# bluecube/minipath

Measured on AMD Instinct MI355X. Metric: Mrays/s, higher is better.
Workload: dtype f32; 1 GPU; atrium stand-in for the absent data/Sponza (reference .gitmodules:1-3: un-fetched submodule), 258432 triangles, generator seed 1; 1920x1080 256spp tile64 seed0x5eed depth1 (reference semantics: primary ray + |d.n|, worker.rs:51-66); parallelism=tiles round-robin over 1 rank(s)

## Files before the change

minipath_amd/csrc/family_launch.h:

```cpp
#pragma once

#include <hip/hip_runtime.h>

#include <string>
#include <type_traits>

#include "launch_plan.h"
#include "mp_internal.h"

namespace mp {

#pragma GCC visibility push(hidden)
int check(hipError_t e, const char* what, std::string& err);
void note_launch(KernelId id);
int launched(KernelId id, std::string& err);
int launch_tiles(const RenderLaunch& L, const LaunchPlan& plan, hipStream_t st, std::string& err);
int launch_paths(const RenderLaunch& L, const LaunchPlan& plan, hipStream_t st, std::string& err);
int launch_aov(const RenderLaunch& L, const mp_aov_planes_ex& planes, const LaunchPlan& plan, hipStream_t st, std::string& err);
int launch_staged(const RenderLaunch& L, const WavefrontPlan& plan, hipStream_t st, std::string& err);
int launch_rays(QueryKind kind, const DevScene& sc, const float* ox, const float* oy, const float* oz, const float* dx, const float* dy,
                const float* dz, const float* tmax, uint64_t n, const mp_hits_soa* hits, uint8_t* occluded, int cu_count, void* stream,
                std::string& err);
#ifdef MP_PROF_MISSES
constexpr int kProfSlots = 10;
int prof_add_tiles(unsigned long long* sum, int reset);
int prof_add_aov(unsigned long long* sum, int reset);
int prof_add_paths(unsigned long long* sum, int reset);
#endif
#pragma GCC visibility pop

#define MP_LAUNCH(id, kernel, grid, block, lds, stream, ...)               \
    do {                                                                   \
        note_launch(id);                                                   \
        hipLaunchKernelGGL(kernel, grid, block, lds, stream, __VA_ARGS__); \
    } while (0)

#define MP_LAUNCH_ROW(row, ...)                                                          \
    case row:                                                                            \
        if constexpr (std::is_invocable_v<decltype(&__VA_ARGS__), Args...>) {            \
            MP_LAUNCH(row, (__VA_ARGS__), dim3(grid), dim3(block), lds, st, args...);    \
            return launched(row, err);                                                   \
        }                                                                                \
        break;
#define MP_FAMILY_LAUNCHER(SUBTABLE)                                                                                              \
    template <class... Args>                                                                                                      \
    int launch(KernelId id, uint32_t grid, uint32_t block, uint32_t lds, hipStream_t st, std::string& err, const Args&... args) { \
        switch (id) {                                                                                                             \
            SUBTABLE(MP_LAUNCH_ROW)                                                                                               \
            default: break;                                                                                                       \
        }                                                                                                                         \
        err = "kernel table: no such kernel for these arguments";                                                                 \
        return MP_ERR_INVALID;                                                                                                    \
    }

namespace {

template <class Plan>
int refused(const Plan& plan, std::string& err) {
    err = plan.error;
    return plan.rc;
}

}
}
```

minipath_amd/csrc/mask_cache.h:

```cpp
#pragma once

#include <hip/hip_runtime.h>

#include <cfloat>
#include <cmath>
#include <cstdint>

#include "camera_rays.h"

#ifndef MP_PROF_COUNT
#define MP_PROF_COUNT(i) do { } while (0)
#endif

namespace mp {
namespace mc {
__device__ __forceinline__ float as_f(uint32_t u) { return __uint_as_float(u); }
__device__ __forceinline__ uint32_t as_u(float f) { return __float_as_uint(f); }

__device__ __forceinline__ void wave_lds_sync() {
    __builtin_amdgcn_fence(__ATOMIC_RELEASE, "wavefront");
    __builtin_amdgcn_wave_barrier();
    __builtin_amdgcn_fence(__ATOMIC_ACQUIRE, "wavefront");
}

struct Ray {
    float ox, oy, oz, dx, dy, dz, ix, iy, iz;
};

__device__ __forceinline__ float fma_dot(float ax, float ay, float az, float bx, float by, float bz) {
    return __builtin_fmaf(az, bz, __builtin_fmaf(ay, by, ax * bx));
}
__device__ __forceinline__ float fms(float a, float b, float c) { return __builtin_fmaf(a, b, -c); }

template <bool PATCH_NAN, int OCT>
__device__ __forceinline__ void slab(float bnx, float bny, float bnz, float bxx, float bxy, float bxz, const Ray& r,
                                     float limit, float& t1, float& t2) {
    float ax = (bnx - r.ox) * r.ix, ay = (bny - r.oy) * r.iy, az = (bnz - r.oz) * r.iz;
    float cx = (bxx - r.ox) * r.ix, cy = (bxy - r.oy) * r.iy, cz = (bxz - r.oz) * r.iz;
    if (PATCH_NAN) {
        ax = fmaxf(ax, -INFINITY); ay = fmaxf(ay, -INFINITY); az = fmaxf(az, -INFINITY);
        cx = fminf(cx, INFINITY); cy = fminf(cy, INFINITY); cz = fminf(cz, INFINITY);
    }
    float lox, loy, loz, hix, hiy, hiz;
    if (OCT >= 0) {
        lox = (OCT & 1) ? cx : ax; hix = (OCT & 1) ? ax : cx;
        loy = (OCT & 2) ? cy : ay; hiy = (OCT & 2) ? ay : cy;
        loz = (OCT & 4) ? cz : az; hiz = (OCT & 4) ? az : cz;
    } else {
        lox = fminf(ax, cx); loy = fminf(ay, cy); loz = fminf(az, cz);
        hix = fmaxf(ax, cx); hiy = fmaxf(ay, cy); hiz = fmaxf(az, cz);
    }
    t1 = fmaxf(fmaxf(lox, 0.0f), fmaxf(loy, loz));
    t2 = fminf(fminf(hix, limit), fminf(hiy, hiz));
}

#ifndef MP_MCACHE_PAD
#define MP_MCACHE_PAD 0.25f
#endif
#ifndef MP_NODE_ENTRIES
#define MP_NODE_ENTRIES 64
#endif
#ifndef MP_LEAF_ENTRIES
#define MP_LEAF_ENTRIES 128
#endif
#ifndef MP_ARENA_ENTRIES
#define MP_ARENA_ENTRIES 384
#endif
#ifndef MP_ARENA_ROOM
#define MP_ARENA_ROOM 384
#endif
#ifndef MP_NODE_SLOT_MASK
#define MP_NODE_SLOT_MASK 0xFFFFFFFFu
#endif
constexpr int kMaskCacheEntries = MP_NODE_ENTRIES;
constexpr int kMaskCacheHeader = 32;
constexpr int kLeafCacheEntries = MP_LEAF_ENTRIES;
constexpr int kLeafTagBase = kMaskCacheHeader + kMaskCacheEntries;
constexpr int kLeafMaskBase = kLeafTagBase + kLeafCacheEntries;
constexpr int kNodeListBase = kLeafMaskBase + 2 * kLeafCacheEntries;
constexpr int kArenaBase = kNodeListBase + kMaskCacheEntries;
constexpr int kArenaRoom = MP_ARENA_ROOM;
constexpr int kArenaEntries = MP_ARENA_ENTRIES;
constexpr int kMaskCacheDwords = kArenaBase + kArenaRoom;
constexpr int kArenaTopSlot = kMaskCacheHeader + kMaskCacheEntries - 1;
constexpr int kRootListSlot = kNodeListBase + kMaskCacheEntries - 1;
static_assert((kMaskCacheEntries & (kMaskCacheEntries - 1)) == 0 && kMaskCacheEntries >= 4, "the node table's slot mask");
static_assert(kArenaEntries >= 16 && kArenaEntries <= kArenaRoom, "an unexpanded list (at most 16 entries) fits the empty arena");
static_assert((kLeafMaskBase % 2) == 0 && (kMaskCacheDwords % 4) == 0, "LDS alignment of the leaf masks / of the next wave's header");
constexpr float kCoordCap = 1073741824.0f;
struct MaskCache {
    uint32_t* lds;
};
#define MP_DPP_STEP6(CTRL)                                                                                              \
    "v_min_f32_dpp %0, %0, %0 " CTRL "\n\tv_min_f32_dpp %1, %1, %1 " CTRL "\n\tv_min_f32_dpp %2, %2, %2 " CTRL "\n\t"         \
    "v_max_f32_dpp %3, %3, %3 " CTRL "\n\tv_max_f32_dpp %4, %4, %4 " CTRL "\n\tv_max_f32_dpp %5, %5, %5 " CTRL "\n\t"
__device__ __forceinline__ void wave_min3_max3(float (&mn)[3], float (&mx)[3]) {
    asm volatile("s_nop 1\n\t"
                 MP_DPP_STEP6("quad_perm:[1,0,3,2] row_mask:0xf bank_mask:0xf")
                 MP_DPP_STEP6("quad_perm:[2,3,0,1] row_mask:0xf bank_mask:0xf")
                 MP_DPP_STEP6("row_half_mirror row_mask:0xf bank_mask:0xf")
                 MP_DPP_STEP6("row_mirror row_mask:0xf bank_mask:0xf")
                 MP_DPP_STEP6("row_bcast:15 row_mask:0xa bank_mask:0xf")
                 MP_DPP_STEP6("row_bcast:31 row_mask:0xc bank_mask:0xf")
                 : "+v"(mn[0]), "+v"(mn[1]), "+v"(mn[2]), "+v"(mx[0]), "+v"(mx[1]), "+v"(mx[2]));
}
__device__ __forceinline__ bool mask_cache_ray_ok(const Ray& r) {
    constexpr uint32_t kMag = 0x7FFFFFFFu;
    const uint32_t mo = max(max(as_u(r.ox) & kMag, as_u(r.oy) & kMag), as_u(r.oz) & kMag);
    const uint32_t mi = max(max(as_u(r.ix) & kMag, as_u(r.iy) & kMag), as_u(r.iz) & kMag);
    const uint32_t md = max(max(as_u(r.dx) & kMag, as_u(r.dy) & kMag), as_u(r.dz) & kMag);
    constexpr uint32_t kCapO = 0x4E800000u , kCapI = 0x7F7FFFFFu , kCapD = 0x40000000u ;
    static_assert(kCoordCap == 1073741824.0f, "kCapO is kCoordCap's bit pattern");
    return static_cast<int32_t>((mo - (kCapO + 1u)) & (mi - (kCapI + 1u)) & (md - (kCapD + 1u))) < 0;
}
constexpr int kHdrState = 12;
constexpr int hdr_lo(int g) { return g == 2 ? kHdrState + 1 : g * 6; }
__device__ __forceinline__ float bounds_deviation(float v, float lo, float hi) {
    return fabsf(v - __builtin_amdgcn_fmed3f(v, lo, hi));
}
__device__ __forceinline__ void mask_cache_begin_pass(const MaskCache& mc, const Ray& r, bool active, uint32_t oct) {
    const int lane = static_cast<int>(threadIdx.x) & 63;
    float* hdr = reinterpret_cast<float*>(mc.lds);
    float h[20];
#pragma unroll
    for (int i = 0; i < 5; i++) {
        const float4 q = reinterpret_cast<const float4*>(mc.lds)[i];
        h[4 * i] = q.x; h[4 * i + 1] = q.y; h[4 * i + 2] = q.z; h[4 * i + 3] = q.w;
    }
    const uint32_t state = __builtin_amdgcn_readfirstlane(as_u(h[kHdrState]));
    const bool same = state == (oct | 0x100u);
    const float val[3][3] = {{r.ox, r.oy, r.oz}, {r.ix, r.iy, r.iz}, {r.dx, r.dy, r.dz}};
    float dev = 0.0f;
#pragma unroll
    for (int g = 0; g < 3; g++) {
#pragma unroll
        for (int k = 0; k < 3; k++) dev = fmaxf(dev, bounds_deviation(val[g][k], h[hdr_lo(g) + k], h[hdr_lo(g) + 3 + k]));
    }
    if (__ballot(active && (!same || dev != 0.0f)) != 0) {
        float pmin[3][3], pmax[3][3];
#pragma unroll
        for (int g = 0; g < 3; g++) {
#pragma unroll
            for (int k = 0; k < 3; k++) {
                pmin[g][k] = active ? val[g][k] : INFINITY;
                pmax[g][k] = active ? val[g][k] : -INFINITY;
            }
            wave_min3_max3(pmin[g], pmax[g]);
        }
#pragma unroll
        for (int g = 0; g < 3; g++) {
#pragma unroll
            for (int k = 0; k < 3; k++) {
                float lo = pmin[g][k], hi = pmax[g][k];
                if (same) { lo = fminf(lo, h[hdr_lo(g) + k]); hi = fmaxf(hi, h[hdr_lo(g) + 3 + k]); }
                const float pad = (hi - lo) * MP_MCACHE_PAD;
                float wlo = lo - pad, whi = hi + pad;
                if (g == 1) {
                    if ((wlo < 0.0f) != (lo < 0.0f) || wlo == 0.0f) wlo = lo;
                    if ((whi < 0.0f) != (hi < 0.0f) || whi == 0.0f) whi = hi;
                    if (!(fabsf(wlo) < INFINITY)) wlo = lo;
                    if (!(fabsf(whi) < INFINITY)) whi = hi;
                } else {
                    const float cap = g == 0 ? 2.0f * kCoordCap : 2.0f;
                    wlo = fmaxf(wlo, -cap); whi = fminf(whi, cap);
                }
                pmin[g][k] = wlo; pmax[g][k] = whi;
            }
        }
        MP_PROF_COUNT(3);
        wave_lds_sync();
        if (lane == 63) {
// ... 258 lines not shown
```

minipath_amd/csrc/mask_probe.hip:

```cpp
#include <hip/hip_runtime.h>

#include <cfloat>
#include <cstdint>

#include "mask_cache.h"

namespace {

using namespace mp::mc;

constexpr int kCounters = 8;
constexpr float kOrgCap = 2.0f * kCoordCap;

__device__ __forceinline__ uint64_t mix64(uint64_t z) {
    z = (z ^ (z >> 30)) * 0xbf58476d1ce4e5b9ull;
    z = (z ^ (z >> 27)) * 0x94d049bb133111ebull;
    return z ^ (z >> 31);
}
__device__ __forceinline__ uint64_t hsh(uint64_t seed, uint64_t c, uint32_t k) { return mix64(seed ^ mix64(c * 0x10000ull + k)); }
__device__ __forceinline__ float unit(uint64_t h) { return static_cast<float>(static_cast<uint32_t>(h >> 40)) * 0x1p-24f; }

__device__ __forceinline__ void record_case(unsigned long long* out, bool bad, uint64_t idx, bool hit, bool rejected, bool edge_only) {
    if ((threadIdx.x & 63) != 0) return;
    atomicAdd(out + 1, 1ull);
// ... 543 lines not shown
                bad = bad || !(nh[k] >= -kOrgCap && nh[k] <= nh[3 + k] && nh[3 + k] <= kOrgCap);
                bad = bad || !(nh[13 + k] >= -2.0f && nh[13 + k] <= nh[16 + k] && nh[16 + k] <= 2.0f);
            }
        }
        bool lane_bad = false;
        for (int g = 0; g < 3; g++)
            for (int k = 0; k < 3; k++) lane_bad = lane_bad || (active && !(val[g * 3 + k] >= nh[hdr_lo(g) + k] && val[g * 3 + k] <= nh[hdr_lo(g) + 3 + k]));
        for (int i = 0; i < kEntryDwords / 64; i++) {
            const uint32_t e = base[kMaskCacheHeader + i * 64 + static_cast<int>(lane)];
            const bool cleared = rewrite && i < (kLeafMaskBase - kMaskCacheHeader) / 64;
            lane_bad = lane_bad || e != (cleared ? 0xFFFFFFFFu : entry_val(seed, c, i, lane));
        }
        bad = bad || __ballot(lane_bad) != 0;
        if (lane == 0u) {
            atomicAdd(out + 1, 1ull);
            if (rewrite) atomicAdd(out + 6, 1ull);
            if (bad) { atomicAdd(out + 0, 1ull); atomicMin(out + 2, static_cast<unsigned long long>(c)); }
        }
        wave_lds_sync();
    }
}

constexpr int kUnitOut = 20;
struct SamplerArg {
    mp_camera_sampler s;
};
__global__ void __launch_bounds__(256) unit_kernel(SamplerArg cam, float jitter_scale, const uint32_t* blocks, uint32_t n, uint32_t* out) {
    __shared__ __align__(16) uint32_t lds[4 * kMaskCacheDwords];
    const uint32_t w = threadIdx.x >> 6, lane = threadIdx.x & 63u;
    const uint32_t unit = blockIdx.x * 4u + w;
    if (unit >= n) return;
    uint32_t* const base = lds + w * kMaskCacheDwords;
    if (lane < static_cast<uint32_t>(kMaskCacheHeader)) base[lane] = static_cast<uint32_t>(hsh(0x0E17ull, unit, lane));
    constexpr int kTags = kLeafMaskBase - kMaskCacheHeader;
    for (int i = 0; i < kTags / 64; i++) base[kMaskCacheHeader + i * 64 + static_cast<int>(lane)] = static_cast<uint32_t>(i * 64) + lane;
    wave_lds_sync();
    mask_cache_begin_unit(MaskCache{base}, cam.s, jitter_scale, blocks[4 * unit], blocks[4 * unit + 1], blocks[4 * unit + 2], blocks[4 * unit + 3]);
    wave_lds_sync();
    uint32_t cleared = 0u;
    for (int i = 0; i < kTags / 64; i++) cleared += static_cast<uint32_t>(__popcll(__ballot(base[kMaskCacheHeader + i * 64 + static_cast<int>(lane)] == 0xFFFFFFFFu)));
    if (lane < 19u) out[kUnitOut * unit + lane] = base[lane];
    if (lane == 19u) out[kUnitOut * unit + 19u] = cleared;
}

constexpr int kListOut = 4 + kArenaRoom;
template <int OCT>
__device__ __noinline__ uint32_t list_slow(const float4* __restrict__ recs, uint32_t* mcache, uint32_t node, uint32_t slots) {
    return unit_list_build(recs, mcache, node, slots,
                           [](const float* b, const float bmn[3], const float bmx[3]) { return bounds_may_hit<OCT>(b, bmn, bmx); });
}
__global__ void __launch_bounds__(256) list_kernel(const float4* recs, uint32_t slots, const uint32_t* headers, const uint32_t* cases, uint32_t n,
                                                   uint32_t* out) {
    __shared__ __align__(16) uint32_t lds[4 * kMaskCacheDwords];
    const uint32_t w = threadIdx.x >> 6, lane = threadIdx.x & 63u;
    const uint32_t c = blockIdx.x * 4u + w;
    if (c >= n) return;
    uint32_t* const base = lds + w * kMaskCacheDwords;
    for (uint32_t i = lane; i < static_cast<uint32_t>(kMaskCacheDwords); i += 64u)
        base[i] = i < static_cast<uint32_t>(kMaskCacheHeader) ? headers[32u * c + i] : i < static_cast<uint32_t>(kLeafMaskBase) ? 0xFFFFFFFFu : 0xDEAD0000u + i;
    wave_lds_sync();
    const uint32_t node = cases[2u * c], top0 = cases[2u * c + 1u];
    if (lane == 0u) base[kArenaTopSlot] = ~top0;
    wave_lds_sync();
    uint32_t val;
    switch (__builtin_amdgcn_readfirstlane(base[kHdrState]) & 7u) {
        case 0: val = list_slow<0>(recs, base, node, slots); break;
        case 1: val = list_slow<1>(recs, base, node, slots); break;
        case 2: val = list_slow<2>(recs, base, node, slots); break;
        case 3: val = list_slow<3>(recs, base, node, slots); break;
        case 4: val = list_slow<4>(recs, base, node, slots); break;
        case 5: val = list_slow<5>(recs, base, node, slots); break;
        case 6: val = list_slow<6>(recs, base, node, slots); break;
        default: val = list_slow<7>(recs, base, node, slots); break;
    }
    wave_lds_sync();
    uint32_t* const o = out + static_cast<size_t>(c) * kListOut;
    if (lane == 0u) {
        const uint32_t slot = node_slot(node);
        o[0] = val; o[1] = ~base[kArenaTopSlot]; o[2] = base[static_cast<uint32_t>(kMaskCacheHeader) + slot]; o[3] = base[static_cast<uint32_t>(kNodeListBase) + slot];
    }
    for (uint32_t i = lane; i < static_cast<uint32_t>(kArenaRoom); i += 64u) o[4u + i] = base[static_cast<uint32_t>(kArenaBase) + i];
}

template <class F>
int run(F launch, unsigned long long* host) {
    (void)hipGetLastError();
    unsigned long long* dev = nullptr;
    unsigned long long init[kCounters] = {0ull, 0ull, ~0ull, 0ull, 0ull, 0ull, 0ull, 0ull};
    hipError_t e = hipMalloc(&dev, sizeof(init));
    if (e != hipSuccess) return static_cast<int>(e);
    e = hipMemcpy(dev, init, sizeof(init), hipMemcpyHostToDevice);
    if (e == hipSuccess) {
        launch(dev);
        e = hipGetLastError();
        if (e == hipSuccess) e = hipDeviceSynchronize();
        if (e == hipSuccess) e = hipMemcpy(host, dev, sizeof(init), hipMemcpyDeviceToHost);
    }
    const hipError_t ef = hipFree(dev);
    return static_cast<int>(e != hipSuccess ? e : ef);
}
void merge(unsigned long long* acc, const unsigned long long* r) {
    for (int i = 0; i < kCounters; i++) if (i != 2) acc[i] += r[i];
    if (r[2] < acc[2]) acc[2] = r[2];
}
void reset(unsigned long long* acc) {
    for (int i = 0; i < kCounters; i++) acc[i] = 0ull;
    acc[2] = ~0ull;
}
constexpr uint64_t kCasesPerLaunch = 1ull << 20;

template <class K>
int run_cases(K kernel, uint64_t seed, uint64_t ncases, uint32_t* dump_dev, unsigned long long* out) {
    unsigned long long acc[kCounters];
    reset(acc);
    for (uint64_t c0 = 0; c0 < ncases; c0 += kCasesPerLaunch) {
        const uint64_t n = ncases - c0 < kCasesPerLaunch ? ncases - c0 : kCasesPerLaunch;
        unsigned long long r[kCounters];
        if (int rc = run([&](unsigned long long* d) {
                hipLaunchKernelGGL(kernel, dim3(static_cast<uint32_t>((n + 3) / 4)), dim3(256), 0, 0, seed, c0, c0 + n, d, dump_dev);
            }, r))
            return rc;
        merge(acc, r);
    }
    for (int i = 0; i < kCounters; i++) out[i] = acc[i];
    return 0;
}

}

extern "C" {
int mp_mask_probe_tri(uint64_t seed, uint64_t ncases, unsigned long long* out) { return run_cases(tri_kernel, seed, ncases, nullptr, out); }
int mp_mask_probe_exits(uint64_t seed, uint64_t ncases, unsigned long long* out) { return run_cases(exit_kernel, seed, ncases, nullptr, out); }
int mp_mask_probe_box(uint64_t seed, uint64_t ncases, unsigned long long* out) { return run_cases(box_kernel, seed, ncases, nullptr, out); }
int mp_mask_probe_dump_dwords() { return kDumpCase; }
int mp_mask_probe_dump(int kind, uint64_t seed, uint64_t ncases, uint32_t* host, unsigned long long* out) {
    (void)hipGetLastError();
    uint32_t* dev = nullptr;
    const size_t bytes = static_cast<size_t>(ncases) * kDumpCase * sizeof(uint32_t);
    hipError_t e = hipMalloc(&dev, bytes);
    if (e != hipSuccess) return static_cast<int>(e);
    e = hipMemset(dev, 0, bytes);
    int rc = static_cast<int>(e);
    if (e == hipSuccess) rc = kind == 0 ? run_cases(tri_kernel, seed, ncases, dev, out) : run_cases(box_kernel, seed, ncases, dev, out);
    if (rc == 0) rc = static_cast<int>(hipMemcpy(host, dev, bytes, hipMemcpyDeviceToHost));
    const hipError_t ef = hipFree(dev);
    return rc != 0 ? rc : static_cast<int>(ef);
}
int mp_mask_probe_ray_ok(uint64_t seed, unsigned long long* out) {
    unsigned long long acc[kCounters];
    reset(acc);
    constexpr uint64_t kThreads = (1ull << 32) / kOkPerThread, kBlocks = kThreads / 256;
    for (int comp = 0; comp < 9; comp++) {
        unsigned long long r[kCounters];
        if (int rc = run([&](unsigned long long* d) {
                hipLaunchKernelGGL(ray_ok_kernel, dim3(static_cast<uint32_t>(kBlocks)), dim3(256), 0, 0, seed, comp, 0ull, d);
            }, r))
            return rc;
        if (r[2] != ~0ull) r[2] += static_cast<unsigned long long>(comp) << 32;
        merge(acc, r);
    }
    for (int i = 0; i < kCounters; i++) out[i] = acc[i];
    return 0;
}
int mp_mask_probe_dev(uint64_t seed, const float* set, uint32_t n, uint64_t nrandom, unsigned long long* out) {
    (void)hipGetLastError();
    float* dset = nullptr;
    hipError_t e = hipMalloc(&dset, sizeof(float) * (n ? n : 1u));
    if (e != hipSuccess) return static_cast<int>(e);
    e = hipMemcpy(dset, set, sizeof(float) * n, hipMemcpyHostToDevice);
    int rc = static_cast<int>(e);
    unsigned long long acc[kCounters];
    reset(acc);
    const uint64_t ntrip = static_cast<uint64_t>(n) * n * n;
    if (rc == 0 && ntrip) {
        unsigned long long r[kCounters];
        rc = run([&](unsigned long long* d) {
            hipLaunchKernelGGL(dev_kernel, dim3(static_cast<uint32_t>((ntrip + 255) / 256)), dim3(256), 0, 0, seed, 0, 0ull, n, dset, d);
        }, r);
        if (rc == 0) merge(acc, r);
    }
    if (rc == 0 && nrandom) {
        unsigned long long r[kCounters];
        rc = run([&](unsigned long long* d) {
            hipLaunchKernelGGL(dev_kernel, dim3(static_cast<uint32_t>((nrandom + 255) / 256)), dim3(256), 0, 0, seed, 1, 0ull, n, dset, d);
        }, r);
        if (rc == 0) { if (r[2] != ~0ull) r[2] += 1ull << 40; merge(acc, r); }
    }
    const hipError_t ef = hipFree(dset);
    if (rc != 0) return rc;
    for (int i = 0; i < kCounters; i++) out[i] = acc[i];
    return static_cast<int>(ef);
}
int mp_mask_probe_unit(const float* sampler, float jitter_scale, const uint32_t* blocks, uint32_t n, uint32_t* out, uint32_t* ntags,
                       float* margin) {
    (void)hipGetLastError();
    *ntags = static_cast<uint32_t>(kLeafMaskBase - kMaskCacheHeader);
    *margin = MP_MCACHE_MARGIN;
    if (n == 0u) return 0;
    SamplerArg cam;
    const float* p = sampler;
    for (int k = 0; k < 3; k++) { cam.s.center[k] = p[k]; cam.s.up[k] = p[3 + k]; cam.s.right[k] = p[6 + k]; cam.s.film_origin_offset[k] = p[9 + k]; }
    cam.s.pixel_scale = p[12]; cam.s.lens_radius = p[13]; cam.s.lens_weight = p[14];
    uint32_t *dblocks = nullptr, *dout = nullptr;
    hipError_t e = hipMalloc(&dblocks, sizeof(uint32_t) * 4u * n);
    if (e == hipSuccess) e = hipMalloc(&dout, sizeof(uint32_t) * kUnitOut * n);
    if (e == hipSuccess) e = hipMemcpy(dblocks, blocks, sizeof(uint32_t) * 4u * n, hipMemcpyHostToDevice);
    if (e == hipSuccess) {
        hipLaunchKernelGGL(unit_kernel, dim3((n + 3u) / 4u), dim3(256), 0, 0, cam, jitter_scale, dblocks, n, dout);
        e = hipGetLastError();
        if (e == hipSuccess) e = hipDeviceSynchronize();
        if (e == hipSuccess) e = hipMemcpy(out, dout, sizeof(uint32_t) * kUnitOut * n, hipMemcpyDeviceToHost);
    }
    (void)hipFree(dblocks);
    (void)hipFree(dout);
    return static_cast<int>(e);
}
int mp_mask_probe_pass(uint64_t seed, uint64_t nwaves, unsigned long long* out) {
    return run([&](unsigned long long* d) {
        hipLaunchKernelGGL(pass_kernel, dim3(static_cast<uint32_t>(nwaves / 4)), dim3(256), 0, 0, seed, d);
    }, out);
}
int mp_mask_probe_list_dwords() { return kListOut; }
int mp_mask_probe_list(const uint32_t* recs, uint32_t n_nodes, uint32_t slots, const uint32_t* headers, const uint32_t* cases, uint32_t ncases,
                       uint32_t* out, uint32_t* info) {
    (void)hipGetLastError();
    if (info) { info[0] = static_cast<uint32_t>(kArenaEntries); info[1] = static_cast<uint32_t>(kMaskCacheEntries); info[2] = static_cast<uint32_t>(kArenaBase); }
    if (slots != 8u && slots != 16u) return -1;
    for (uint32_t c = 0; c < ncases; c++)
        if (cases[2u * c] >= n_nodes || cases[2u * c + 1u] > static_cast<uint32_t>(kArenaEntries)) return -1;
    for (size_t i = 0; i < static_cast<size_t>(n_nodes) * slots; i++) {
        const uint32_t link = recs[i * 8u + 6u];
        if (link != kNullLink && (link & 63u) == 0u && (link >> 6) >= n_nodes) return -1;
    }
    if (ncases == 0u) return 0;
    uint32_t *drecs = nullptr, *dhdr = nullptr, *dcases = nullptr, *dout = nullptr;
    const size_t rec_bytes = sizeof(uint32_t) * 8u * slots * n_nodes, out_bytes = sizeof(uint32_t) * kListOut * static_cast<size_t>(ncases);
    hipError_t e = hipMalloc(&drecs, rec_bytes);
    if (e == hipSuccess) e = hipMalloc(&dhdr, sizeof(uint32_t) * 32u * ncases);
    if (e == hipSuccess) e = hipMalloc(&dcases, sizeof(uint32_t) * 2u * ncases);
    if (e == hipSuccess) e = hipMalloc(&dout, out_bytes);
    if (e == hipSuccess) e = hipMemcpy(drecs, recs, rec_bytes, hipMemcpyHostToDevice);
    if (e == hipSuccess) e = hipMemcpy(dhdr, headers, sizeof(uint32_t) * 32u * ncases, hipMemcpyHostToDevice);
    if (e == hipSuccess) e = hipMemcpy(dcases, cases, sizeof(uint32_t) * 2u * ncases, hipMemcpyHostToDevice);
    if (e == hipSuccess) {
        hipLaunchKernelGGL(list_kernel, dim3((ncases + 3u) / 4u), dim3(256), 0, 0, reinterpret_cast<const float4*>(drecs), slots, dhdr, dcases, ncases, dout);
        e = hipGetLastError();
        if (e == hipSuccess) e = hipDeviceSynchronize();
        if (e == hipSuccess) e = hipMemcpy(out, dout, out_bytes, hipMemcpyDeviceToHost);
    }
    (void)hipFree(drecs); (void)hipFree(dhdr); (void)hipFree(dcases); (void)hipFree(dout);
    return static_cast<int>(e);
}
}
```

minipath_amd/csrc/packet_walk.h:

```cpp
#pragma once

#include "prof_counters.h"

#include "group_walk.h"
#include "launch_plan.h"

namespace mp {
namespace {

typedef const __attribute__((address_space(4))) float* kfp;
typedef const __attribute__((address_space(4))) uint32_t* kup;
typedef float krec8 __attribute__((ext_vector_type(8)));

constexpr float kTiny = 9.094947017729282e-13f;
constexpr float kHuge = 1099511627776.0f;


struct PacketHit {
    float t, u, v;
    uint32_t prim;
};

constexpr uint32_t kSrcRoot = 0xFFFFFFFFu;

// ... 148 lines not shown
                a0 = nd[16]; a1 = nd[17]; a2 = nd[18]; a3 = nd[19]; a4 = nd[20]; a5 = nd[21]; a6 = nd[22];
                child(b0, b1, b2, b3, b4, b5, b6, slot + 1u);
                slot += 2u;
                nd += 16;
            }
            if (nchild & 1u) child(a0, a1, a2, a3, a4, a5, a6, slot);
            st.sync(sp);
        } else {
            const uint32_t first = link >> 6, n_real = link & 63u;
            kfp tp = tris + static_cast<size_t>(first) * (8 * kTriDwords);
            const float thr = on ? -kTiny : INFINITY;
            uint64_t changed = 0;
            auto test = [&](const float v0x, const float v0y, const float v0z, const float e1x, const float e1y, const float e1z,
                            const float e2x, const float e2y, const float e2z, const uint32_t tri) {
                const float hx = fms(r.dy, e2z, r.dz * e2y), hy = fms(r.dz, e2x, r.dx * e2z), hz = fms(r.dx, e2y, r.dy * e2x);
                const float det = fma_dot(e1x, e1y, e1z, hx, hy, hz);
                const float sx = r.ox - v0x, sy = r.oy - v0y, sz = r.oz - v0z;
                const float un = fma_dot(sx, sy, sz, hx, hy, hz);
                const uint32_t det_sign = as_u(det) & 0x80000000u;
                const bool det_ok = fabsf(det) <= kHuge;
                const float xu = det_ok ? as_f(as_u(un) ^ det_sign) : 1.0f;
                if (__ballot(!(xu <= thr)) == 0) return;
                const float qx = fms(sy, e1z, sz * e1y), qy = fms(sz, e1x, sx * e1z), qz = fms(sx, e1y, sy * e1x);
                const float vn = fma_dot(r.dx, r.dy, r.dz, qx, qy, qz);
                const float tn = fma_dot(e2x, e2y, e2z, qx, qy, qz);
                const float xv = det_ok ? as_f(as_u(vn) ^ det_sign) : 1.0f, xt = det_ok ? as_f(as_u(tn) ^ det_sign) : 1.0f;
                if (__ballot(!(fminf(fminf(xu, xv), xt) <= thr)) == 0) return;
                const float inv_det = 1.0f / det;
                const float u = inv_det * un, v = inv_det * vn, t = inv_det * tn;
                const bool acc = (u >= 0.0f) & (v >= 0.0f) & ((u + v) <= 1.0f) & (t >= 0.0f) & (t < lim);
                best_t = acc ? t : best_t;
                lim = acc ? t : lim;
                bu = acc ? u : bu;
                bv = acc ? v : bv;
                bprim = acc ? tri : bprim;
                changed |= __ballot(acc);
            };
            float a0 = tp[0], a1 = tp[1], a2 = tp[2], a3 = tp[3], a4 = tp[4], a5 = tp[5], a6 = tp[6], a7 = tp[7], a8 = tp[8];
            uint32_t tri = first * 8u;
            for (uint32_t p = n_real >> 1; p > 0; p--) {
                const float b0 = tp[9], b1 = tp[10], b2 = tp[11], b3 = tp[12], b4 = tp[13], b5 = tp[14], b6 = tp[15], b7 = tp[16], b8 = tp[17];
                test(a0, a1, a2, a3, a4, a5, a6, a7, a8, tri);
                a0 = tp[18]; a1 = tp[19]; a2 = tp[20]; a3 = tp[21]; a4 = tp[22]; a5 = tp[23]; a6 = tp[24]; a7 = tp[25]; a8 = tp[26];
                test(b0, b1, b2, b3, b4, b5, b6, b7, b8, tri + 1u);
                tri += 2u;
                tp += 2 * kTriDwords;
            }
            if (n_real & 1u) test(a0, a1, a2, a3, a4, a5, a6, a7, a8, tri);
            if (changed != 0) stale_top = sp;
        }
    }
    hit.t = best_t; hit.u = bu; hit.v = bv; hit.prim = bprim;
}

struct RegStack3 {
    int ent, mlo, mhi;
    __device__ __forceinline__ RegStack3() : ent(0), mlo(0), mhi(0) {}
    __device__ __forceinline__ void push(int sp, uint32_t e, uint64_t m) {
        asm volatile("s_mov_b32 m0, %3\n\ts_nop 0\n\t"
                     "v_writelane_b32 %0, %4, m0\n\tv_writelane_b32 %1, %5, m0\n\tv_writelane_b32 %2, %6, m0"
                     : "+v"(ent), "+v"(mlo), "+v"(mhi)
                     : "s"(sp), "s"(e), "s"(static_cast<uint32_t>(m)), "s"(static_cast<uint32_t>(m >> 32))
                     : "m0");
    }
    __device__ __forceinline__ void pop(int sp, uint32_t& e, uint64_t& m) const {
        e = static_cast<uint32_t>(__builtin_amdgcn_readlane(ent, sp));
        m = static_cast<uint32_t>(__builtin_amdgcn_readlane(mlo, sp)) |
            (static_cast<uint64_t>(static_cast<uint32_t>(__builtin_amdgcn_readlane(mhi, sp))) << 32);
    }
};

template <int OCT>
__device__ __noinline__ uint32_t unit_list_slow(const float* __restrict__ nodes_pk, uint32_t* mcache, uint32_t node, uint32_t slots) {
    return unit_list_build(reinterpret_cast<const float4*>(nodes_pk), mcache, node, slots,
                           [](const float* b, const float bmn[3], const float bmx[3]) { return bounds_may_hit<OCT>(b, bmn, bmx); });
}
template <int OCT>
__device__ __forceinline__ bool trace_packet_cached(const DevScene& sc, const Ray& r, bool active, PacketHit& hit, uint32_t* mcache) {
    static_assert(kNullLink == MP_LINK_NULL, "mask_cache.h's copy of the null link");
    kfp nodes = (kfp)(uintptr_t)sc.nodes_pk;
    kfp tris = (kfp)(uintptr_t)sc.tris_aos;
    float best_t = FLT_MAX, bu = 0.0f, bv = 0.0f;
    uint32_t bprim = kNoPrim;
    RegStack3 st;
    int sp = 0;
    mcache[kRootListSlot] = sc.pk_count * sc.pk_mask_bits;
    wave_lds_sync();
    uint32_t cur = (static_cast<uint32_t>(kRootListSlot) << 16) | 1u;
    uint64_t pm = __ballot(active);
    for (;;) {
        if ((cur & 0xFFFFu) == 0u) {
            if (sp == 0) break;
            sp--;
            st.pop(sp, cur, pm);
        }
        cur -= 1u;
        const uint32_t src = __builtin_amdgcn_readfirstlane(mcache[(cur >> 16) + (cur & 0xFFFFu)]);
#ifndef MP_NO_EMPTY_SKIP
        if (static_cast<int32_t>(src) < 0) {
            MP_PROF_COUNT(7);
            continue;
        }
#endif
        const bool pon = __builtin_amdgcn_inverse_ballot_w64(pm);
        const krec8 rec = *reinterpret_cast<const __attribute__((address_space(4))) krec8*>(reinterpret_cast<const __attribute__((address_space(4))) char*>(nodes) + scalar_u(src * 32u));
        float t1, t2;
        slab<false, OCT>(rec[0], rec[1], rec[2], rec[3], rec[4], rec[5], r, pon ? best_t : -1.0f, t1, t2);
        const bool ok = t1 <= t2;
        if (__ballot(ok) == 0) continue;
        const uint32_t link = uniform_u(rec[6]);
        float lim = ok ? best_t : -1.0f;
        if ((link & 63u) == 0u) {
            MP_PROF_COUNT(2);
            const uint32_t node = link >> 6;
            const uint32_t slot = node_slot(node);
            const uint32_t tag = __builtin_amdgcn_readfirstlane(mcache[static_cast<uint32_t>(kMaskCacheHeader) + slot]);
            uint32_t list = __builtin_amdgcn_readfirstlane(mcache[static_cast<uint32_t>(kNodeListBase) + slot]);
            if (__builtin_expect(tag != node, 0)) {
                MP_PROF_COUNT(0);
                if (tag != 0xFFFFFFFFu) MP_PROF_COUNT(4);
                list = __builtin_amdgcn_readfirstlane(unit_list_slow<OCT>(sc.nodes_pk, mcache, node, sc.pk_mask_bits));
                if (list == kListOverflow) {
                    if (sp != 0 || (cur & 0xFFFFu) != 0u) {
                        MP_PROF_COUNT(6);
                        return false;
                    }
                    list = __builtin_amdgcn_readfirstlane(unit_list_slow<OCT>(sc.nodes_pk, mcache, node, sc.pk_mask_bits));
                }
            }
            if ((list & 0xFFFFu) != 0u) {
                if ((cur & 0xFFFFu) != 0u) {
                    st.push(sp, cur, pm);
                    sp++;
                }
                cur = list;
                pm = __ballot(lim >= 0.0f);
            }
        } else {
            const uint32_t first = link >> 6, n_real = link & 63u;
            kfp tp = tris + static_cast<size_t>(first) * (8 * kTriDwords);
            static_assert(kExitTiny == kTiny && kExitHuge == kHuge, "mask_cache.h's copies of the early-out constants");
            const float thr = lim >= 0.0f ? -kTiny : INFINITY;
            auto test = [&](const float v0x, const float v0y, const float v0z, const float e1x, const float e1y, const float e1z,
                            const float e2x, const float e2y, const float e2z, const uint32_t tri) {
                const float hx = fms(r.dy, e2z, r.dz * e2y), hy = fms(r.dz, e2x, r.dx * e2z), hz = fms(r.dx, e2y, r.dy * e2x);
                const float det = fma_dot(e1x, e1y, e1z, hx, hy, hz);
                const float sx = r.ox - v0x, sy = r.oy - v0y, sz = r.oz - v0z;
                const float un = fma_dot(sx, sy, sz, hx, hy, hz);
                const float xu = tri_flipped(det, un);
                if (__ballot(!(tri_exit1_key(det, xu) <= thr)) == 0) return;
                const float qx = fms(sy, e1z, sz * e1y), qy = fms(sz, e1x, sx * e1z), qz = fms(sx, e1y, sy * e1x);
                const float vn = fma_dot(r.dx, r.dy, r.dz, qx, qy, qz);
                const float tn = fma_dot(e2x, e2y, e2z, qx, qy, qz);
                const float xv = tri_flipped(det, vn), xt = tri_flipped(det, tn);
                if (__ballot(!(tri_exit2_key(det, xu, xv, xt) <= thr)) == 0) return;
                constexpr uint32_t kRcpLo = 0x10800000u , kRcpHi = 0x7E000000u ;
                const uint32_t wkey = (as_u(det) << 1) - (kRcpLo << 1);
                const float inv_det = __ballot(wkey > ((kRcpHi - kRcpLo) << 1)) == 0 ? rm::rcp_short(det) : 1.0f / det;
                const float u = inv_det * un, v = inv_det * vn, t = inv_det * tn;
                const bool acc = !(fminf(fminf(u, v), t) < 0.0f) & ((u + v) <= 1.0f) & (t < lim);
                best_t = acc ? t : best_t;
                lim = acc ? t : lim;
                bu = acc ? u : bu;
                bv = acc ? v : bv;
                bprim = acc ? tri : bprim;
            };
            const uint32_t ls = first & static_cast<uint32_t>(kLeafCacheEntries - 1);
            const uint32_t tag = mcache[kLeafTagBase + ls];
            const uint2 tm = reinterpret_cast<const uint2*>(mcache + kLeafMaskBase)[ls];
            uint64_t todo;
            if (__builtin_expect(__builtin_amdgcn_readfirstlane(tag) == first, 1)) {
                todo = __builtin_amdgcn_readfirstlane(tm.x) | (static_cast<uint64_t>(__builtin_amdgcn_readfirstlane(tm.y)) << 32);
            } else {
                MP_PROF_COUNT(1);
                const uint64_t m = leaf_mask_slow(sc.tris_aos, mcache, first, n_real);
                todo = __builtin_amdgcn_readfirstlane(static_cast<uint32_t>(m)) | (static_cast<uint64_t>(__builtin_amdgcn_readfirstlane(static_cast<uint32_t>(m >> 32))) << 32);
            }
#ifndef MP_NO_EMPTY_SKIP
            if (todo == 0 && (cur >> 16) != static_cast<uint32_t>(kRootListSlot)) {
                if ((threadIdx.x & 63u) == 0u) mcache[(cur >> 16) + (cur & 0xFFFFu)] = src | kEmptyLeafBit;
                wave_lds_sync();
            }
#endif
            if (todo != 0) {
                uint32_t c = static_cast<uint32_t>(__builtin_ctzll(todo));
                todo &= ~(1ull << c);
                kfp ta = tri_record(tp, c);
                krec8 ra = *reinterpret_cast<const __attribute__((address_space(4))) krec8*>(ta);
                float a8 = ta[8];
                while (todo != 0) {
                    const uint32_t cn = static_cast<uint32_t>(__builtin_ctzll(todo));
                    todo &= ~(1ull << cn);
                    kfp tb = tri_record(tp, cn);
                    const krec8 rb = *reinterpret_cast<const __attribute__((address_space(4))) krec8*>(tb);
                    const float b8 = tb[8];
                    test(ra[0], ra[1], ra[2], ra[3], ra[4], ra[5], ra[6], ra[7], a8, first * 8u + c);
                    ra = rb; a8 = b8;
                    c = cn;
                }
                test(ra[0], ra[1], ra[2], ra[3], ra[4], ra[5], ra[6], ra[7], a8, first * 8u + c);
            }
        }
    }
    hit.t = best_t; hit.u = bu; hit.v = bv; hit.prim = bprim;
    return true;
}

template <bool OCTANTS, class Stack, bool MC = false>
__device__ __forceinline__ void trace_packet(const DevScene& sc, const Ray& r, bool active, Stack& st, PacketHit& hit,
                                             const MaskCache& mc = MaskCache{nullptr}) {
    if (OCTANTS && MC) {
        if (__ballot(active & !mask_cache_ray_ok(r)) != 0) {
            const bool slow = active && (fabsf(r.ix) == INFINITY || fabsf(r.iy) == INFINITY || fabsf(r.iz) == INFINITY);
            if (__ballot(slow) != 0) trace_packet_impl<2, -1>(sc, r, active, st, hit);
            else trace_packet_impl<1, -1>(sc, r, active, st, hit);
            return;
        }
    } else {
        const bool slow = active && (fabsf(r.ix) == INFINITY || fabsf(r.iy) == INFINITY || fabsf(r.iz) == INFINITY);
        if (__ballot(slow) != 0) {
            trace_packet_impl<2, -1>(sc, r, active, st, hit);
            return;
        }
    }
    if (OCTANTS && sc.boxes_ordered) {
        const uint64_t am = __ballot(active);
        const uint64_t nx = __ballot(active && r.ix < 0.0f), ny = __ballot(active && r.iy < 0.0f), nz = __ballot(active && r.iz < 0.0f);
        if ((nx == 0 || nx == am) && (ny == 0 || ny == am) && (nz == 0 || nz == am)) {
            const uint32_t oct = (nx ? 1u : 0u) | (ny ? 2u : 0u) | (nz ? 4u : 0u);
            if (MC) {
                mask_cache_begin_pass(mc, r, active, oct);
                bool done;
                switch (oct) {
                    case 0: done = trace_packet_cached<0>(sc, r, active, hit, mc.lds); break;
                    case 1: done = trace_packet_cached<1>(sc, r, active, hit, mc.lds); break;
                    case 2: done = trace_packet_cached<2>(sc, r, active, hit, mc.lds); break;
                    case 3: done = trace_packet_cached<3>(sc, r, active, hit, mc.lds); break;
                    case 4: done = trace_packet_cached<4>(sc, r, active, hit, mc.lds); break;
                    case 5: done = trace_packet_cached<5>(sc, r, active, hit, mc.lds); break;
                    case 6: done = trace_packet_cached<6>(sc, r, active, hit, mc.lds); break;
                    default: done = trace_packet_cached<7>(sc, r, active, hit, mc.lds); break;
                }
                if (done) return;
            } else {
                switch (oct) {
                    case 0: trace_packet_impl<1, 0>(sc, r, active, st, hit); return;
                    case 1: trace_packet_impl<1, 1>(sc, r, active, st, hit); return;
                    case 2: trace_packet_impl<1, 2>(sc, r, active, st, hit); return;
                    case 3: trace_packet_impl<1, 3>(sc, r, active, st, hit); return;
                    case 4: trace_packet_impl<1, 4>(sc, r, active, st, hit); return;
                    case 5: trace_packet_impl<1, 5>(sc, r, active, st, hit); return;
                    case 6: trace_packet_impl<1, 6>(sc, r, active, st, hit); return;
                    default: trace_packet_impl<1, 7>(sc, r, active, st, hit); return;
                }
            }
        }
    }
    trace_packet_impl<1, -1>(sc, r, active, st, hit);
}

template <class T>
__device__ __forceinline__ const T* uniform_ptr(const T* p) {
    const uint64_t v = reinterpret_cast<uint64_t>(p);
    const uint32_t lo = __builtin_amdgcn_readfirstlane(static_cast<uint32_t>(v)), hi = __builtin_amdgcn_readfirstlane(static_cast<uint32_t>(v >> 32));
    return reinterpret_cast<const T*>((static_cast<uint64_t>(hi) << 32) | lo);
}

// ... 33 lines not shown
```

minipath_amd/csrc/prof_counters.h:

```cpp
#pragma once

#ifdef MP_PROF_MISSES
#ifdef MP_PROF_COUNT
#error "prof_counters.h comes before mask_cache.h: include packet_walk.h first"
#endif
#include <hip/hip_runtime.h>

#include "family_launch.h"

namespace mp {
namespace {
__device__ unsigned long long g_prof[10];
static_assert(sizeof(g_prof) / sizeof(g_prof[0]) == kProfSlots, "family_launch.h's count of the slots");

inline int prof_add_unit(unsigned long long* sum, int reset) {
    unsigned long long all[kProfSlots] = {};
    if (hipMemcpyFromSymbol(all, HIP_SYMBOL(g_prof), sizeof(all)) != hipSuccess) return 1;
    for (int i = 0; i < kProfSlots; i++) sum[i] += all[i];
    if (reset) {
        const unsigned long long z[kProfSlots] = {};
        if (hipMemcpyToSymbol(HIP_SYMBOL(g_prof), z, sizeof(z)) != hipSuccess) return 1;
    }
    return 0;
}
}
}
#define MP_PROF_COUNT(i) do { if ((threadIdx.x & 63u) == 0u) atomicAdd(&g_prof[i], 1ull); } while (0)
#endif
```

Baseline: 39090 Mrays/s.

## Move packet-walk traversal stack into LDS frames and defer leaf limit setup

The packet walk's register stack (RegStack3) is replaced by a small per-wave frame array in the LDS mask-cache header, holding up to four frames by default. Each frame stores the cursor and the 64-bit packet mask, and is read back with readfirstlane so the values stay uniform. This frees registers, which may raise occupancy. The per-lane limit/threshold computation is also deferred until a leaf actually has triangles to test, reusing the ballot mask as the child packet mask. The cost is a fixed stack depth: an overflow returns false, presumably falling back to another path. A probe kernel for testing the frames is added.

Result: no change. 39460 Mrays/s (median of 6 runs) (+1.0%).

```diff
diff --git a/minipath_amd/csrc/family_launch.h b/minipath_amd/csrc/family_launch.h
--- a/minipath_amd/csrc/family_launch.h
+++ b/minipath_amd/csrc/family_launch.h
@@ -22,7 +22,7 @@
                 const float* dz, const float* tmax, uint64_t n, const mp_hits_soa* hits, uint8_t* occluded, int cu_count, void* stream,
                 std::string& err);
 #ifdef MP_PROF_MISSES
-constexpr int kProfSlots = 10;
+constexpr int kProfSlots = 12;
 int prof_add_tiles(unsigned long long* sum, int reset);
 int prof_add_aov(unsigned long long* sum, int reset);
 int prof_add_paths(unsigned long long* sum, int reset);
diff --git a/minipath_amd/csrc/mask_cache.h b/minipath_amd/csrc/mask_cache.h
--- a/minipath_amd/csrc/mask_cache.h
+++ b/minipath_amd/csrc/mask_cache.h
@@ -71,6 +71,9 @@
 #endif
 #ifndef MP_NODE_SLOT_MASK
 #define MP_NODE_SLOT_MASK 0xFFFFFFFFu
+#endif
+#ifndef MP_FRAME_SLOTS
+#define MP_FRAME_SLOTS 4
 #endif
 constexpr int kMaskCacheEntries = MP_NODE_ENTRIES;
 constexpr int kMaskCacheHeader = 32;
@@ -87,6 +90,26 @@
 static_assert((kMaskCacheEntries & (kMaskCacheEntries - 1)) == 0 && kMaskCacheEntries >= 4, "the node table's slot mask");
 static_assert(kArenaEntries >= 16 && kArenaEntries <= kArenaRoom, "an unexpanded list (at most 16 entries) fits the empty arena");
 static_assert((kLeafMaskBase % 2) == 0 && (kMaskCacheDwords % 4) == 0, "LDS alignment of the leaf masks / of the next wave's header");
+constexpr int kFrameSlots = MP_FRAME_SLOTS;
+constexpr int kFrameBase = kFrameSlots <= 4 ? 20 : kArenaBase + kArenaRoom - 3 * kFrameSlots;
+static_assert(kFrameSlots >= 1, "the walk's frame array");
+static_assert(kFrameSlots <= 4 || kArenaEntries + 3 * kFrameSlots <= kArenaRoom, "more than four frames: MP_ARENA_ENTRIES makes room for them");
+static_assert(kFrameBase > 18 && (kFrameSlots > 4 || kFrameBase + 3 * kFrameSlots <= kMaskCacheHeader), "frames overlap neither B nor the tags");
+__device__ __forceinline__ bool frame_push(uint32_t* mcache, uint32_t& fp, uint32_t cur, uint64_t pm) {
+    if (fp == static_cast<uint32_t>(3 * kFrameSlots)) return false;
+    uint32_t* f = mcache + static_cast<uint32_t>(kFrameBase) + fp;
+    f[0] = cur; f[1] = static_cast<uint32_t>(pm); f[2] = static_cast<uint32_t>(pm >> 32);
+    fp += 3u;
+    return true;
+}
+__device__ __forceinline__ void frame_pop(const uint32_t* mcache, uint32_t& fp, uint32_t& cur, uint64_t& pm) {
+    fp -= 3u;
+    const uint32_t* f = mcache + static_cast<uint32_t>(kFrameBase) + fp;
+    const uint32_t a = f[0], b = f[1], c = f[2];
+    cur = static_cast<uint32_t>(__builtin_amdgcn_readfirstlane(a));
+    pm = static_cast<uint32_t>(__builtin_amdgcn_readfirstlane(b)) | (static_cast<uint64_t>(static_cast<uint32_t>(__builtin_amdgcn_readfirstlane(c))) << 32);
+}
+
 constexpr float kCoordCap = 1073741824.0f;
 struct MaskCache {
     uint32_t* lds;
diff --git a/minipath_amd/csrc/mask_probe.hip b/minipath_amd/csrc/mask_probe.hip
--- a/minipath_amd/csrc/mask_probe.hip
+++ b/minipath_amd/csrc/mask_probe.hip
@@ -649,6 +649,45 @@
     for (uint32_t i = lane; i < static_cast<uint32_t>(kArenaRoom); i += 64u) o[4u + i] = base[static_cast<uint32_t>(kArenaBase) + i];
 }
 
+constexpr int kFrameTries = kFrameSlots + 1;
+constexpr int kFrameOut = 4 + 3 * kFrameTries;
+__device__ __forceinline__ void frame_case(uint32_t w, uint32_t k, uint32_t& cur, uint64_t& pm) {
+    cur = __builtin_amdgcn_readfirstlane(0xC0DE0000u ^ (w << 12) ^ (k * 0x01010101u + 1u));
+    const uint64_t m = mix64((static_cast<uint64_t>(w) << 32) | k) | 1ull;
+    pm = static_cast<uint32_t>(__builtin_amdgcn_readfirstlane(static_cast<uint32_t>(m))) |
+         (static_cast<uint64_t>(static_cast<uint32_t>(__builtin_amdgcn_readfirstlane(static_cast<uint32_t>(m >> 32)))) << 32);
+}
+__global__ void __launch_bounds__(256) frames_kernel(const uint32_t* counts, uint32_t* out) {
+    __shared__ __align__(16) uint32_t lds[4 * kMaskCacheDwords];
+    const uint32_t w = __builtin_amdgcn_readfirstlane(threadIdx.x >> 6), lane = threadIdx.x & 63u;
+    for (uint32_t i = threadIdx.x; i < 4u * static_cast<uint32_t>(kMaskCacheDwords); i += 256u) lds[i] = 0xA5000000u + i;
+    __syncthreads();
+    uint32_t* const base = lds + w * kMaskCacheDwords;
+    uint32_t* const o = out + w * kFrameOut;
+    const uint32_t n = min(__builtin_amdgcn_readfirstlane(counts[w]), static_cast<uint32_t>(kFrameTries));
+    uint32_t fp = 0u, accepted = 0u, refused = 0xFFFFFFFFu;
+    for (uint32_t k = 0; k < n; k++) {
+        uint32_t cur;
+        uint64_t pm;
+        frame_case(w, k, cur, pm);
+        if (frame_push(base, fp, cur, pm)) accepted++;
+        else if (refused == 0xFFFFFFFFu) refused = k;
+    }
+    if (lane == 0u) { o[0] = accepted; o[1] = refused; o[2] = fp; }
+    __syncthreads();
+    for (uint32_t i = threadIdx.x; i < 4u * static_cast<uint32_t>(kMaskCacheDwords); i += 256u) out[4 * kFrameOut + i] = lds[i];
+    __syncthreads();
+    uint32_t k = 0u;
+    while (fp != 0u) {
+        uint32_t cur;
+        uint64_t pm;
+        frame_pop(base, fp, cur, pm);
+        if (lane == 0u) { o[4 + 3 * k] = cur; o[5 + 3 * k] = static_cast<uint32_t>(pm); o[6 + 3 * k] = static_cast<uint32_t>(pm >> 32); }
+        k++;
+    }
+    if (lane == 0u) o[3] = fp;
+}
+
 template <class F>
 int run(F launch, unsigned long long* host) {
     (void)hipGetLastError();
@@ -787,6 +826,26 @@
         hipLaunchKernelGGL(pass_kernel, dim3(static_cast<uint32_t>(nwaves / 4)), dim3(256), 0, 0, seed, d);
     }, out);
 }
+int mp_mask_probe_frames_dwords() { return 4 * kFrameOut + 4 * kMaskCacheDwords; }
+int mp_mask_probe_frames(const uint32_t* counts, uint32_t* out, uint32_t* info) {
+    (void)hipGetLastError();
+    info[0] = static_cast<uint32_t>(kFrameSlots); info[1] = static_cast<uint32_t>(kFrameBase); info[2] = static_cast<uint32_t>(kMaskCacheDwords);
+    info[3] = static_cast<uint32_t>(kFrameOut);
+    uint32_t *dcounts = nullptr, *dout = nullptr;
+    const size_t out_bytes = sizeof(uint32_t) * static_cast<size_t>(mp_mask_probe_frames_dwords());
+    hipError_t e = hipMalloc(&dcounts, sizeof(uint32_t) * 4u);
+    if (e == hipSuccess) e = hipMalloc(&dout, out_bytes);
+    if (e == hipSuccess) e = hipMemset(dout, 0, out_bytes);
+    if (e == hipSuccess) e = hipMemcpy(dcounts, counts, sizeof(uint32_t) * 4u, hipMemcpyHostToDevice);
+    if (e == hipSuccess) {
+        hipLaunchKernelGGL(frames_kernel, dim3(1), dim3(256), 0, 0, dcounts, dout);
+        e = hipGetLastError();
+        if (e == hipSuccess) e = hipDeviceSynchronize();
+        if (e == hipSuccess) e = hipMemcpy(out, dout, out_bytes, hipMemcpyDeviceToHost);
+    }
+    (void)hipFree(dcounts); (void)hipFree(dout);
+    return static_cast<int>(e);
+}
 int mp_mask_probe_list_dwords() { return kListOut; }
 int mp_mask_probe_list(const uint32_t* recs, uint32_t n_nodes, uint32_t slots, const uint32_t* headers, const uint32_t* cases, uint32_t ncases,
                        uint32_t* out, uint32_t* info) {
diff --git a/minipath_amd/csrc/packet_walk.h b/minipath_amd/csrc/packet_walk.h
--- a/minipath_amd/csrc/packet_walk.h
+++ b/minipath_amd/csrc/packet_walk.h
@@ -254,8 +254,12 @@
     kfp tris = (kfp)(uintptr_t)sc.tris_aos;
     float best_t = FLT_MAX, bu = 0.0f, bv = 0.0f;
     uint32_t bprim = kNoPrim;
+#ifdef MP_NO_LDS_FRAMES
     RegStack3 st;
     int sp = 0;
+#else
+    uint32_t sp = 0u;
+#endif
     mcache[kRootListSlot] = sc.pk_count * sc.pk_mask_bits;
     wave_lds_sync();
     uint32_t cur = (static_cast<uint32_t>(kRootListSlot) << 16) | 1u;
@@ -263,8 +267,12 @@
     for (;;) {
         if ((cur & 0xFFFFu) == 0u) {
             if (sp == 0) break;
+#ifdef MP_NO_LDS_FRAMES
             sp--;
             st.pop(sp, cur, pm);
+#else
+            frame_pop(mcache, sp, cur, pm);
+#endif
         }
         cur -= 1u;
         const uint32_t src = __builtin_amdgcn_readfirstlane(mcache[(cur >> 16) + (cur & 0xFFFFu)]);
@@ -278,10 +286,12 @@
         const krec8 rec = *reinterpret_cast<const __attribute__((address_space(4))) krec8*>(reinterpret_cast<const __attribute__((address_space(4))) char*>(nodes) + scalar_u(src * 32u));
         float t1, t2;
         slab<false, OCT>(rec[0], rec[1], rec[2], rec[3], rec[4], rec[5], r, pon ? best_t : -1.0f, t1, t2);
-        const bool ok = t1 <= t2;
-        if (__ballot(ok) == 0) continue;
+        const uint64_t okm = __ballot(t1 <= t2);
+        if (okm == 0) continue;
         const uint32_t link = uniform_u(rec[6]);
-        float lim = ok ? best_t : -1.0f;
+#ifdef MP_NO_LATE_LIM
+        float lim = __builtin_amdgcn_inverse_ballot_w64(okm) ? best_t : -1.0f;
+#endif
         if ((link & 63u) == 0u) {
             MP_PROF_COUNT(2);
             const uint32_t node = link >> 6;
@@ -302,17 +312,34 @@
             }
             if ((list & 0xFFFFu) != 0u) {
                 if ((cur & 0xFFFFu) != 0u) {
+                    MP_PROF_COUNT(10);
+#ifdef MP_NO_LDS_FRAMES
                     st.push(sp, cur, pm);
                     sp++;
+#else
+                    if (__builtin_expect(!frame_push(mcache, sp, cur, pm), 0)) {
+                        MP_PROF_COUNT(11);
+                        MP_PROF_COUNT(6);
+                        return false;
+                    }
+#endif
                 }
                 cur = list;
+#ifdef MP_NO_LATE_LIM
                 pm = __ballot(lim >= 0.0f);
+#else
+                pm = okm;
+#endif
             }
         } else {
             const uint32_t first = link >> 6, n_real = link & 63u;
             kfp tp = tris + static_cast<size_t>(first) * (8 * kTriDwords);
             static_assert(kExitTiny == kTiny && kExitHuge == kHuge, "mask_cache.h's copies of the early-out constants");
+#ifdef MP_NO_LATE_LIM
             const float thr = lim >= 0.0f ? -kTiny : INFINITY;
+#else
+            float lim, thr;
+#endif
             auto test = [&](const float v0x, const float v0y, const float v0z, const float e1x, const float e1y, const float e1z,
                             const float e2x, const float e2y, const float e2z, const uint32_t tri) {
                 const float hx = fms(r.dy, e2z, r.dz * e2y), hy = fms(r.dz, e2x, r.dx * e2z), hz = fms(r.dx, e2y, r.dy * e2x);
@@ -355,6 +382,11 @@
             }
 #endif
             if (todo != 0) {
+#ifndef MP_NO_LATE_LIM
+                const bool live = __builtin_amdgcn_inverse_ballot_w64(okm);
+                lim = live ? best_t : -1.0f;
+                thr = live ? -kTiny : INFINITY;
+#endif
                 uint32_t c = static_cast<uint32_t>(__builtin_ctzll(todo));
                 todo &= ~(1ull << c);
                 kfp ta = tri_record(tp, c);
diff --git a/minipath_amd/csrc/prof_counters.h b/minipath_amd/csrc/prof_counters.h
--- a/minipath_amd/csrc/prof_counters.h
+++ b/minipath_amd/csrc/prof_counters.h
@@ -10,7 +10,7 @@
 
 namespace mp {
 namespace {
-__device__ unsigned long long g_prof[10];
+__device__ unsigned long long g_prof[12];
 static_assert(sizeof(g_prof) / sizeof(g_prof[0]) == kProfSlots, "family_launch.h's count of the slots");
 
 inline int prof_add_unit(unsigned long long* sum, int reset) {
```
